# AlexanderKazakov/gcm

Hardware: AMD Instinct MI355X
Metric: Mnode-steps/sec + achieved HBM GB/s, 3D isotropic elastic 512³ CubicGrid (higher is better)
Workload: dtype f64; 1 GPU; 3-D isotropic elastic CubicGrid 512^3, borderSize 2, Courant 0.9, tau 0.9, one full time step (3 stages); global_nodes=134217728, slabs=1, launch=single process, parallelism=single, fp=fma

## Files before the change

gcm_amd/csrc/iso.hpp:

```cpp
#pragma once

#include "common.hpp"
#include "launch.hpp"

namespace gcmx {


__host__ __device__ constexpr int sig3(int i, int j) {
	return (i <= j) ? 3 + (i * 3 - ((i - 1) * i) / 2 + j - i)
	                : 3 + (j * 3 - ((j - 1) * j) / 2 + i - j);
}
__host__ __device__ constexpr unsigned bit(int i) { return 1u << i; }

__host__ __device__ constexpr int tang1(int s) { return s == 0 ? 1 : 0; }
__host__ __device__ constexpr int tang2(int s) { return s == 2 ? 1 : 2; }
__host__ __device__ constexpr int sgn1(int s) { return s == 0 ? -1 : 1; }
__host__ __device__ constexpr int sgn2(int s) { return s == 2 ? 1 : -1; }

enum Slot : int { kZero = 0, kOne, kHalf, kA, kB, kG, kP1, kP2, kS };
struct Coef {
	int slot;
	int sign;
};
__host__ __device__ constexpr Coef cz() { return Coef{kZero, 0}; }
// ... 3 lines not shown
	const int ss = sig3(S, S), st1 = sig3(t1, S), st2 = sig3(t2, S);
	const int s11 = sig3(t1, t1), s22 = sig3(t2, t2), s12 = sig3(t1, t2);
	return (k == 0) ? (j == S ? Coef{kOne, 1} : j == ss ? Coef{kA, 1} : cz())
	     : (k == 1) ? (j == S ? Coef{kOne, 1} : j == ss ? Coef{kA, -1} : cz())
	     : (k == 2) ? (j == t1 ? Coef{kOne, s1} : j == st1 ? Coef{kB, s1} : cz())
	     : (k == 3) ? (j == t1 ? Coef{kOne, s1} : j == st1 ? Coef{kB, -s1} : cz())
	     : (k == 4) ? (j == t2 ? Coef{kOne, s2} : j == st2 ? Coef{kB, s2} : cz())
	     : (k == 5) ? (j == t2 ? Coef{kOne, s2} : j == st2 ? Coef{kB, -s2} : cz())
	     : (k == 6) ? (j == s12 ? Coef{kOne, s1 * s2} : cz())
	     : (k == 7) ? (j == s11 ? Coef{kOne, 1} : j == s22 ? Coef{kOne, -1} : cz())
	                : (j == s11 ? Coef{kOne, 1} : j == s22 ? Coef{kOne, 1}
	                   : j == ss ? Coef{kG, 1} : cz());
}

__host__ __device__ constexpr Coef iso_u1(int S, int c, int n) {
	const int t1 = tang1(S), t2 = tang2(S), s1 = sgn1(S), s2 = sgn2(S);
	const int ss = sig3(S, S), st1 = sig3(t1, S), st2 = sig3(t2, S);
	const int s11 = sig3(t1, t1), s22 = sig3(t2, t2), s12 = sig3(t1, t2);
	return (n == 0) ? (c == S ? Coef{kHalf, 1} : c == ss ? Coef{kP1, 1}
	                   : (c == s11 || c == s22) ? Coef{kP2, 1} : cz())
	     : (n == 1) ? (c == S ? Coef{kHalf, 1} : c == ss ? Coef{kP1, -1}
	                   : (c == s11 || c == s22) ? Coef{kP2, -1} : cz())
	     : (n == 2) ? (c == t1 ? Coef{kHalf, s1} : c == st1 ? Coef{kS, s1} : cz())
	     : (n == 3) ? (c == t1 ? Coef{kHalf, s1} : c == st1 ? Coef{kS, -s1} : cz())
	     : (n == 4) ? (c == t2 ? Coef{kHalf, s2} : c == st2 ? Coef{kS, s2} : cz())
	     : (n == 5) ? (c == t2 ? Coef{kHalf, s2} : c == st2 ? Coef{kS, -s2} : cz())
	     : (n == 6) ? (c == s12 ? Coef{kOne, s1 * s2} : cz())
	     : (n == 7) ? (c == s11 ? Coef{kHalf, 1} : c == s22 ? Coef{kHalf, -1} : cz())
	                : (c == s11 ? Coef{kHalf, 1} : c == s22 ? Coef{kHalf, 1} : cz());
}

__host__ __device__ constexpr unsigned iso_window(int S) {
	unsigned m = 0;
	for (int k = 0; k < 6; k++)
		for (int j = 0; j < 9; j++)
			if (iso_u(S, k, j).slot != kZero) m |= bit(j);
	return m;
}
__host__ __device__ constexpr unsigned iso_center_only(int S) {
	unsigned m = 0;
	for (int k = 6; k < 9; k++)
		for (int j = 0; j < 9; j++)
			if (iso_u(S, k, j).slot != kZero) m |= bit(j);
	return m & ~iso_window(S);
}
__host__ __device__ constexpr int wslot(unsigned mask, int j) {
	int n = 0;
	for (int i = 0; i < j; i++) n += (mask >> i) & 1u;
	return n;
}
__host__ __device__ constexpr int popc9(unsigned m) {
	int n = 0;
	for (int i = 0; i < 9; i++) n += (m >> i) & 1u;
	return n;
}
template <int SLOT, int SIGN>
__device__ __forceinline__ double term(const IsoAxis& A, double v) {
	double m;
	if constexpr (SLOT == kOne) m = v;
	else if constexpr (SLOT == kHalf) m = v * 0.5;
	else if constexpr (SLOT == kA) m = A.a * v;
	else if constexpr (SLOT == kB) m = A.b * v;
	else if constexpr (SLOT == kG) m = A.g * v;
	else if constexpr (SLOT == kP1) m = A.p1 * v;
	else if constexpr (SLOT == kP2) m = A.p2 * v;
	else m = A.s * v;
	return SIGN > 0 ? m : -m;
}

template <int S, bool ISU1, int ROW, int J = 0>
struct RowSum {
	template <class F>
	__device__ __forceinline__ static double go(const IsoAxis& A, F val, double acc, bool first) {
		if constexpr (J == 9) {
			return acc;
		} else {
			constexpr Coef c = ISU1 ? iso_u1(S, ROW, J) : iso_u(S, ROW, J);
			if constexpr (c.slot == kZero) {
				return RowSum<S, ISU1, ROW, J + 1>::go(A, val, acc, first);
			} else {
				const double t = term<c.slot, c.sign>(A, val(J));
				return RowSum<S, ISU1, ROW, J + 1>::go(A, val, first ? t : acc + t, false);
			}
		}
	}
};

__host__ __device__ constexpr int pair_vel(int S, int P) { return P == 0 ? S : P == 1 ? tang1(S) : tang2(S); }
__host__ __device__ constexpr int pair_sig(int S, int P) {
	return P == 0 ? sig3(S, S) : P == 1 ? sig3(tang1(S), S) : sig3(tang2(S), S);
}

#ifndef GCMX_FMA
#define GCMX_FMA 0
#endif
#ifndef GCMX_LAGRANGE
#define GCMX_LAGRANGE GCMX_FMA
#endif
template <int BS>
__device__ __forceinline__ double lagrange_minmax(const double (&s)[BS + 1], const double* __restrict__ w) {
	double ans = s[0] * w[0];
#pragma unroll
	for (int i = 1; i <= BS; i++) ans = __builtin_fma(w[i], s[i], ans);
	return vlimit(ans, s[0], s[1]);
}

template <int S, int BS, bool KF0, int P, class WF>
__device__ __forceinline__ void pair_update(const IsoAxis& A, WF W, double& ra, double& rb) {
	const double* coef = (P == 0) ? A.c1 : A.c2;
	const double* wts = (P == 0) ? A.w1 : A.w2;
	const int kf = (P == 0) ? A.kf1 : A.kf2;
	auto interp = [&](int j, int sh) {
		double sv[BS + 1];
#pragma unroll
		for (int i = 0; i <= BS; i++) sv[i] = W(j, sh * i);
		if constexpr (GCMX_LAGRANGE && KF0 && BS <= 2) return lagrange_minmax<BS>(sv, wts);
		else return newton_minmax<BS, KF0>(sv, kf, coef);
	};
	ra = RowSum<S, false, 2 * P>::go(A, [&](int j) { return interp(j, -1); }, 0.0, true);
	rb = RowSum<S, false, 2 * P + 1>::go(A, [&](int j) { return interp(j, 1); }, 0.0, true);
}

template <int S, class CF>
__device__ __forceinline__ void center_update(const IsoAxis& A, CF C, double (&r)[9]) {
	r[6] = RowSum<S, false, 6>::go(A, C, 0.0, true);
	r[7] = RowSum<S, false, 7>::go(A, C, 0.0, true);
	r[8] = RowSum<S, false, 8>::go(A, C, 0.0, true);
}

template <int S>
__device__ __forceinline__ void u1_apply(const IsoAxis& A, const double (&r)[9], double (&out)[9]) {
	auto rv = [&](int n) { return r[n]; };
	out[0] = RowSum<S, true, 0>::go(A, rv, 0.0, true);
	out[1] = RowSum<S, true, 1>::go(A, rv, 0.0, true);
	out[2] = RowSum<S, true, 2>::go(A, rv, 0.0, true);
	out[3] = RowSum<S, true, 3>::go(A, rv, 0.0, true);
	out[4] = RowSum<S, true, 4>::go(A, rv, 0.0, true);
	out[5] = RowSum<S, true, 5>::go(A, rv, 0.0, true);
	out[6] = RowSum<S, true, 6>::go(A, rv, 0.0, true);
	out[7] = RowSum<S, true, 7>::go(A, rv, 0.0, true);
	out[8] = RowSum<S, true, 8>::go(A, rv, 0.0, true);
}

template <int S, int BS, bool KF0, class WF, class CF>
__device__ __forceinline__ void node_update(const IsoAxis& A, WF W, CF C, double (&out)[9]) {
	double r[9];
	pair_update<S, BS, KF0, 0>(A, W, r[0], r[1]);
	pair_update<S, BS, KF0, 1>(A, W, r[2], r[3]);
	pair_update<S, BS, KF0, 2>(A, W, r[4], r[5]);
	center_update<S>(A, C, r);
	u1_apply<S>(A, r, out);
}

typedef const __attribute__((address_space(1))) double* gcptr;
typedef __attribute__((address_space(1))) double* gptr;
#ifndef GCMX_SGPR_BASES
#define GCMX_SGPR_BASES 1
#endif
__device__ __forceinline__ gcptr sgpr_ptr(const double* p) {
	gcptr q = (gcptr)p;
#if GCMX_SGPR_BASES
	asm volatile("" : "+s"(q));
#endif
	return q;
}
__device__ __forceinline__ gptr sgpr_ptr(double* p) {
	gptr q = (gptr)p;
#if GCMX_SGPR_BASES
	asm volatile("" : "+s"(q));
#endif
	return q;
}
struct Planes {
	gcptr b[kMaxM];
	__device__ __forceinline__ Planes(const double* p, long long cs) {
#pragma unroll
		for (int j = 0; j < kMaxM; j++) b[j] = sgpr_ptr(p + j * cs);
	}
	__device__ __forceinline__ double ld(int j, unsigned off) const {
		typedef const __attribute__((address_space(1))) char* gcb;
		return *reinterpret_cast<gcptr>(reinterpret_cast<gcb>(b[j]) + (size_t)(off << 3));
	}
};
struct PlanesW {
	gptr b[kMaxM];
	__device__ __forceinline__ PlanesW(double* p, long long cs) {
#pragma unroll
		for (int j = 0; j < kMaxM; j++) b[j] = sgpr_ptr(p + j * cs);
	}
	__device__ __forceinline__ void st(int j, unsigned off, double v) const {
		typedef __attribute__((address_space(1))) char* gb;
		*reinterpret_cast<gptr>(reinterpret_cast<gb>(b[j]) + (size_t)(off << 3)) = v;
	}
	__device__ __forceinline__ void st_nt(int j, unsigned off, double v) const {
		typedef __attribute__((address_space(1))) char* gb;
		__builtin_nontemporal_store(v, reinterpret_cast<gptr>(reinterpret_cast<gb>(b[j]) + (size_t)(off << 3)));
	}
};

__device__ __forceinline__ unsigned opaque_u32(unsigned x) {
	asm("" : "+v"(x));
	return x;
}
__device__ __forceinline__ double ld_b(const Planes& p, int j, unsigned boff) {
	typedef const __attribute__((address_space(1))) char* gcb;
	return *reinterpret_cast<gcptr>(reinterpret_cast<gcb>(p.b[j]) + (unsigned long long)boff);
}
__device__ __forceinline__ double ld_nt_b(const Planes& p, int j, unsigned boff) {
	typedef const __attribute__((address_space(1))) char* gcb;
	return __builtin_nontemporal_load(reinterpret_cast<gcptr>(reinterpret_cast<gcb>(p.b[j]) + (unsigned long long)boff));
}
__device__ __forceinline__ void st_b(const PlanesW& p, int j, unsigned boff, double v) {
	typedef __attribute__((address_space(1))) char* gb;
	*reinterpret_cast<gptr>(reinterpret_cast<gb>(p.b[j]) + (unsigned long long)boff) = v;
}
__device__ __forceinline__ void st_nt_b(const PlanesW& p, int j, unsigned boff, double v) {
	typedef __attribute__((address_space(1))) char* gb;
	__builtin_nontemporal_store(v, reinterpret_cast<gptr>(reinterpret_cast<gb>(p.b[j]) + (unsigned long long)boff));
}

typedef double dpair __attribute__((ext_vector_type(2)));
__device__ __forceinline__ dpair ld2_b(const Planes& p, int j, unsigned boff) {
	typedef const __attribute__((address_space(1))) char* gcb;
	typedef const __attribute__((address_space(1))) dpair* gcp2;
	return *reinterpret_cast<gcp2>(reinterpret_cast<gcb>(p.b[j]) + (unsigned long long)boff);
}
__device__ __forceinline__ dpair ld2_nt_b(const Planes& p, int j, unsigned boff) {
	typedef const __attribute__((address_space(1))) char* gcb;
	typedef const __attribute__((address_space(1))) dpair* gcp2;
	return __builtin_nontemporal_load(reinterpret_cast<gcp2>(reinterpret_cast<gcb>(p.b[j]) + (unsigned long long)boff));
}
__device__ __forceinline__ void st2_b(const PlanesW& p, int j, unsigned boff, dpair v) {
	typedef __attribute__((address_space(1))) char* gb;
	typedef __attribute__((address_space(1))) dpair* gp2;
	*reinterpret_cast<gp2>(reinterpret_cast<gb>(p.b[j]) + (unsigned long long)boff) = v;
}
__device__ __forceinline__ void st2_nt_b(const PlanesW& p, int j, unsigned boff, dpair v) {
	typedef __attribute__((address_space(1))) char* gb;
	typedef __attribute__((address_space(1))) dpair* gp2;
	__builtin_nontemporal_store(v, reinterpret_cast<gp2>(reinterpret_cast<gb>(p.b[j]) + (unsigned long long)boff));
}
__device__ __forceinline__ void half_swap(double& a, double& b) {
	typedef unsigned u32x2 __attribute__((ext_vector_type(2)));
	const u32x2 x = __builtin_bit_cast(u32x2, a), y = __builtin_bit_cast(u32x2, b);
	const u32x2 lo = __builtin_amdgcn_permlane32_swap(x.x, y.x, false, false);
	const u32x2 hi = __builtin_amdgcn_permlane32_swap(x.y, y.y, false, false);
	a = __builtin_bit_cast(double, u32x2{lo.x, hi.x});
	b = __builtin_bit_cast(double, u32x2{lo.y, hi.y});
}

}
```

gcm_amd/csrc/kernels_xyz.hip:

```cpp
#include "iso.hpp"

#include <cstring>
#include <string>
#include <type_traits>

namespace gcmx {
#ifndef GCMX_FMA
#define GCMX_FMA 0
#endif
#if GCMX_FMA
#define GCMX_XYZ_NS xyz_fma
#define GCMX_FP_TAG ", FMA"
#else
#define GCMX_XYZ_NS xyz_exact
#define GCMX_FP_TAG ""
#endif
namespace GCMX_XYZ_NS {


#ifndef GCMX_XYZ_MINWAVES
#define GCMX_XYZ_MINWAVES 4
#endif
#ifndef GCMX_XYZ_CHUNK
#define GCMX_XYZ_CHUNK 128
// ... 111 lines not shown
	};
#pragma unroll
	for (int k = 0; k < W; k++) {
		const int r = yb - BS + k;
		double xr[9];
		if (r >= 0 && r < Y) {
			PairWin wa;
			x_load_a(wa, r);
			x_stage_rest(wa, r, xr);
		} else {
#pragma unroll
			for (int j = 0; j < 9; j++) xr[j] = 0.0;
		}
		push(xr, k);
	}
	auto clamp_row = [&](int r) { return r < Y + BS - 1 ? r : Y + BS - 1; };
	const unsigned zo = live ? (unsigned)z : (unsigned)Z;

	int buf = 0;
#pragma unroll GCMX_XYZ_UNROLL
	for (int y = yb; y < ye; y++) {
		double yv[9];
		node_update<1, BS, KF0>(
		    AY, [&](int j, int o) { return win[wslot(WMY, j)][BS + o]; },
		    [&](int j) { return ((WMY >> j) & 1u) ? win[wslot(WMY, j)][BS] : cen[0][wslot(CMY, j)]; },
		    yv);
#pragma unroll
		for (int j = 0; j < 9; j++)
			if ((WMZ >> j) & 1u) lds[buf][wslot(WMZ, j)][BS + z] = live ? yv[j] : 0.0;
		PairWin wa_next;
		__syncthreads();
		{
			double zv[9];
			node_update<2, BS, KF0>(
			    AZ, [&](int j, int o) { return lds[buf][wslot(WMZ, j)][BS + z + o]; },
			    [&](int j) { return ((WMZ >> j) & 1u) ? lds[buf][wslot(WMZ, j)][BS + z] : yv[j]; }, zv);
			const unsigned offo = plane + (unsigned)y * sty + zo;
			sched_fence();
			x_load_a(wa_next, clamp_row(y + BS + 1));
			sched_fence();
#pragma unroll
			for (int c = 0; c < 9; c++) out_p.st_nt(c, offo, live ? zv[c] : 0.0);
		}
		buf ^= 1;
#pragma unroll
		for (int q = 0; q < NWY; q++)
#pragma unroll
			for (int o = 0; o < W - 1; o++) win[q][o] = win[q][o + 1];
#pragma unroll
		for (int k = 0; k < BS; k++)
#pragma unroll
			for (int q = 0; q < (NCY > 0 ? NCY : 1); q++) cen[k][q] = cen[k + 1][q];
		{
			double xr[9];
			sched_fence();
			x_stage_rest(wa_next, clamp_row(y + BS + 1), xr);
			push(xr, W - 1);
			sched_fence();
		}
	}
}


#ifndef GCMX_TX2_MINWAVES
#define GCMX_TX2_MINWAVES 2
#endif
#ifndef GCMX_TX2_ZS2
#define GCMX_TX2_ZS2 -1
#endif
#ifndef GCMX_TX2_NB
#define GCMX_TX2_NB 1
#endif
#ifndef GCMX_TX2_SLEEP
#define GCMX_TX2_SLEEP 1
#endif
#ifndef GCMX_TX2_BUF
#define GCMX_TX2_BUF 1
#endif
#ifndef GCMX_TX2_PROBE_NOX
#define GCMX_TX2_PROBE_NOX 0
#endif
#ifndef GCMX_TX2_DIAG
#define GCMX_TX2_DIAG 0
#endif
#if GCMX_TX2_DIAG
__device__ unsigned long long g_tx2_diag[16][8];
#define TX2_T(i)                                                      \
	do {                                                              \
		const unsigned long long now_ = __builtin_amdgcn_s_memtime(); \
		dt_[i] += now_ - tprev_;                                      \
		tprev_ = now_;                                                \
	} while (0)
#else
#define TX2_T(i) \
	do {         \
	} while (0)
#endif
#ifndef GCMX_TX2_GEN2_DEFAULT
#define GCMX_TX2_GEN2_DEFAULT 64
#endif
#ifndef GCMX_TX2_PRIO
#define GCMX_TX2_PRIO 0
#endif
#if GCMX_TX2_PRIO
#define TX2_PRIO_HI() __builtin_amdgcn_s_setprio(GCMX_TX2_PRIO)
#define TX2_PRIO_LO() __builtin_amdgcn_s_setprio(0)
#else
#define TX2_PRIO_HI() \
	do {              \
	} while (0)
#define TX2_PRIO_LO() \
	do {              \
	} while (0)
#endif
#ifndef GCMX_TX2_ZPERM
#define GCMX_TX2_ZPERM 1
#endif
#ifndef GCMX_TX2_BLKT
#define GCMX_TX2_BLKT 0
#endif
#if GCMX_TX2_BLKT
constexpr int kBlkMax = 8192;
__device__ unsigned long long g_tx2_blk[kBlkMax][8][2];
__device__ unsigned g_tx2_hw[kBlkMax];
#endif

#ifndef GCMX_TX2_FACEMAP
#define GCMX_TX2_FACEMAP 1
#endif
#ifndef GCMX_TX2_FACE_LDS
#define GCMX_TX2_FACE_LDS 0
#endif
#ifndef GCMX_TX2_STNT
#define GCMX_TX2_STNT 1
#endif
#ifndef GCMX_TX2_ALT
#define GCMX_TX2_ALT 1
#endif
#ifndef GCMX_TX2_NTOUTER
#define GCMX_TX2_NTOUTER 0
#endif
#ifndef GCMX_TX2_NTLOAD
#define GCMX_TX2_NTLOAD 1
#endif
#ifndef GCMX_HET_AB
#define GCMX_HET_AB 0
#endif
#ifndef GCMX_ZS_PAIRS_FIRST
#define GCMX_ZS_PAIRS_FIRST 1
#endif

#ifndef GCMX_TX2_WIDE
#define GCMX_TX2_WIDE 1
#endif
#ifndef GCMX_TX2_UNROLL
#define GCMX_TX2_UNROLL 1
#endif



__host__ __device__ constexpr int wcomp(unsigned mask, int q) {
	int n = 0;
	for (int j = 0; j < 9; j++)
		if ((mask >> j) & 1u) {
			if (n == q) return j;
			n++;
		}
	return -1;
}

template <int BS, int ZT, bool KF0, bool UNI, bool FACES, bool HET, bool ZS = false, bool WD = false>
__global__ __launch_bounds__(ZT, GCMX_TX2_MINWAVES) void k_step_tx2(
    const double* __restrict__ in, double* __restrict__ outl, Geo g, IsoAxis AX, IsoAxis AY_,
    IsoAxis AZ_, int x0, int chunk, int nplanes, int xb0, int nplanesb, FaceBC fb,
    const IsoAxis* __restrict__ mtab, const uint8_t* __restrict__ mat) {
	static_assert(!HET || (KF0 && UNI), "heterogeneous step: floor(q) = 0, Z == ZT, equal axes");
	static_assert(!ZS || (UNI && !HET), "z split: uniform medium");
	const IsoAxis& AY = UNI ? AX : AY_;
	const IsoAxis& AZ = UNI ? AX : AZ_;
	constexpr unsigned WMX = iso_window(0);
	constexpr unsigned CMX = iso_center_only(0);
	constexpr int NCX = popc9(CMX);
	constexpr unsigned WMY = iso_window(1);
	constexpr unsigned CMY = iso_center_only(1);
	constexpr int NWY = popc9(WMY);
	constexpr int NCY = popc9(CMY);
	constexpr unsigned WMZ = iso_window(2);
	constexpr int NWZ = popc9(WMZ);
	constexpr int W = 2 * BS + 1;
	constexpr int WX = W + 1;
	constexpr int LW = ZT + 2 * BS;
	static_assert(NCX >= 1 && NCY >= 1, "isotropic structure");
	constexpr bool NB = UNI && GCMX_TX2_NB;
	constexpr int NW = ZT / 64;
	static_assert(!NB || ZT % 64 == 0, "NB needs whole waves");
	constexpr bool WIDE = WD && NB && GCMX_TX2_WIDE && GCMX_TX2_BUF;
	static_assert(!WD || WIDE, "wide instance launched without its path compiled in");
	constexpr int RW = WIDE ? 68 : 64 + 2 * BS;
	constexpr bool ZS2 = GCMX_TX2_ZS2 < 0 ? !NB : GCMX_TX2_ZS2 != 0;
	__shared__ double zl[NB ? 1 : 2][NB ? 1 : NWZ][NB ? 1 : LW];
	__shared__ double rg[NB ? NW : 1][NB ? 2 : 1][NB ? NWZ : 1][NB ? RW : 1];
	__shared__ double eg[NB ? 2 : 1][NB ? NW : 1][2][NB ? 2 : 1][NB ? NWZ : 1][BS];
	__shared__ int rdy[NB ? NW : 1];
	__shared__ double cl[BS + 1][2][NCY][ZT];
	__shared__ IsoAxis hlds[HET ? kHetMaxMaterials : 1];
	__shared__ double hode[HET ? kHetMaxMaterials : 1];
	__shared__ double flds[FACES && GCMX_TX2_FACE_LDS ? 4 : 1][9];

#if GCMX_TX2_ZPERM
	const int z = [] {
		int w = __builtin_amdgcn_readfirstlane((int)(threadIdx.x >> 6));
		if constexpr (ZT == 512) w = w < 4 ? 2 * w : 2 * (w - 4) + 1;
		const int l = (int)(threadIdx.x & 63);
		return w * 64 + (WIDE ? ((l & 31) << 1) | (l >> 5) : l);
	}();
#else
	const int z = WIDE ? (int)((threadIdx.x & ~63u) | ((threadIdx.x & 31u) << 1) | ((threadIdx.x >> 5) & 1u)) : (int)threadIdx.x;
#endif
#if GCMX_TX2_BLKT
	const unsigned long long blk_t0_ = __builtin_amdgcn_s_memrealtime();
#endif
	const int Y = g.sizes[1], Z = g.sizes[2];
	int x, yb, ye, xbeg, xend;
	bool rev;
	int zp = 0;
	const int nz = ZS ? g.sizes[2] / ZT : 1;
	{
		const int pa = (g.gx0 + x0) & 1, pb = (g.gx0 + xb0) & 1;
		const int npa = (nplanes + pa + 1) / 2;
		const int npair = npa + (nplanesb > 0 ? (nplanesb + pb + 1) / 2 : 0);
		const int T = (int)gridDim.x, b = (int)blockIdx.x;
		int p = xcd_order(b, T);
		if constexpr (ZS && !GCMX_ZS_PAIRS_FIRST) {
			zp = p % nz;
			p /= nz;
		}
		int q = p % npair;
		int cidx = p / npair;
		if (!ZS && chunk < 0) {
			const int co = (-chunk) & 0xFFFF, half = T >> 4;
			const int j = b >> 3, gen = j >= half ? 1 : 0;
			const int G = (b & 7) * half + (j - gen * half);
			const int ncg = (T >> 1) / npair;
			q = G % npair;
			cidx = G / npair + gen * ncg;
			const int cy = (-chunk) >> 16;
			auto start = [&](int c) { return c <= ncg ? c * co : ncg * co + (c - ncg) * cy; };
			yb = start(cidx);
			ye = min(start(cidx + 1), Y);
		}
		x = q < npa ? x0 - pa + 2 * q : xb0 - pb + 2 * (q - npa);
		xbeg = q < npa ? x0 : xb0;
		xend = q < npa ? x0 + nplanes : xb0 + nplanesb;
		if constexpr (ZS && GCMX_ZS_PAIRS_FIRST) {
			zp = cidx % nz;
			cidx /= nz;
		}
		if (ZS || chunk > 0) {
			yb = cidx * chunk;
			ye = min(yb + chunk, Y);
		}
		rev = GCMX_TX2_ALT && (cidx & 1);
	}
	const bool one = x >= xbeg;
	const bool two = x + 1 < xend;
	const bool live = UNI || z < Z;
	const int zc = live ? z : Z - 1;
	const unsigned stx = (unsigned)g.stride[0];
	const unsigned sty = (unsigned)g.stride[1];
	const long long pbase = (long long)x * g.stride[0];
	const unsigned plane = (unsigned)g.origin;
	const unsigned zo = live ? (unsigned)z : (unsigned)Z;
#if GCMX_TX2_BUF
	const Planes src(in + pbase, g.cs);
	const PlanesW out_p(outl + pbase, g.cs);
	const unsigned zpart = ZS ? (unsigned)(zp * ZT) : 0u;
	const int zg = (int)zpart + zc;
	const unsigned lv = (zpart + (unsigned)zc) * 8u, sv = (zpart + zo) * 8u;
	const unsigned pxm = plane - (unsigned)BS * stx;
	auto ldx = [&](int j, int k, int r) {
#if GCMX_TX2_PROBE_NOX
		k = k < BS ? BS : (k > BS + 1 ? BS + 1 : k);
#endif
		const int d = (k == WX - 1 && !two) ? 2 * BS : (k == 0 && !one) ? 1 : k;
		if (GCMX_TX2_NTOUTER && (k == 0 || k == WX - 1))
			return ld_nt_b(src, j, opaque_u32(lv + (pxm + (unsigned)d * stx + (unsigned)r * sty) * 8u));
		return ld_b(src, j, opaque_u32(lv + (pxm + (unsigned)d * stx + (unsigned)r * sty) * 8u));
	};
	auto ldc = [&](int j, int k, int r) {
		if constexpr (!GCMX_TX2_NTLOAD) return ldx(j, k, r);
		const int d = (k == WX - 1 && !two) ? 2 * BS : (k == 0 && !one) ? 1 : k;
		return ld_nt_b(src, j, opaque_u32(lv + (pxm + (unsigned)d * stx + (unsigned)r * sty) * 8u));
	};
	auto stz = [&](int c, int t, int y, double v) {
		const unsigned o = opaque_u32(sv + (plane + (unsigned)t * stx + (unsigned)y * sty) * 8u);
		if constexpr (GCMX_TX2_STNT) st_nt_b(out_p, c, o, v);
		else st_b(out_p, c, o, v);
	};
	const bool hsel = (threadIdx.x & 32u) != 0;
	const unsigned lw = (zpart + (unsigned)(z & ~63) + 2u * (threadIdx.x & 31u)) * 8u;
	auto ldw = [&](int j, int ka, int kb, int r, bool nt) {
		auto cl_ = [&](int k) { return (k == WX - 1 && !two) ? 2 * BS : (k == 0 && !one) ? 1 : k; };
		const unsigned pa = (pxm + (unsigned)cl_(ka) * stx) * 8u, pb = (pxm + (unsigned)cl_(kb) * stx) * 8u;
		const unsigned o = opaque_u32(lw + (hsel ? pb : pa) + (unsigned)r * sty * 8u);
		return nt ? ld2_nt_b(src, j, o) : ld2_b(src, j, o);
	};
	auto stw = [&](int c, int y, double v0, double v1) {
		const unsigned o = opaque_u32(lw + (plane + (hsel ? stx : 0u) + (unsigned)y * sty) * 8u);
		const dpair v = {v0, v1};
		if constexpr (GCMX_TX2_STNT) st2_nt_b(out_p, c, o, v);
		else st2_b(out_p, c, o, v);
	};
#else
	const unsigned base = plane + zc;
	const Planes src(in + pbase, g.cs);
	const PlanesW out_p(outl + pbase, g.cs);
	auto ldx = [&](int j, int k, int r) {
		const int d = (k == WX - 1 && !two) ? BS : (k == 0 && !one) ? 1 - BS : k - BS;
		return src.ld(j, base + (unsigned)r * sty + (unsigned)d * stx);
	};
	auto ldc = [&](int j, int k, int r) { return ldx(j, k, r); };
	auto stz = [&](int c, int t, int y, double v) { out_p.st_nt(c, plane + (unsigned)y * sty + zo + (unsigned)t * stx, v); };
#endif
	auto mt = [&](unsigned k) -> const IsoAxis& {
		if constexpr (GCMX_HET_AB >= 1) return AX;
		return hlds[k];
	};
	auto two_v = [&](int f, int j) -> double {
		if constexpr (FACES && GCMX_TX2_FACE_LDS) return flds[f][j];
		return fb.two_v[f][j];
	};
	struct GhostRule {
		unsigned mask;
		bool none;
		double two[9];
	};
	auto ghost_rule = [&](int f, int t, int pos, unsigned need) -> GhostRule {
		GhostRule r;
		r.none = false;
		if (GCMX_TX2_FACEMAP && fb.map[f]) {
			const int xx = (t == 1 && !two) ? x : (t == 0 && !one) ? x + 1 : x + t;
			const unsigned c = fb.map[f][(size_t)xx * (f < 2 ? Z : Y) + pos];
			r.none = c == kNoFaceCond;
			const FaceCond& fc = fb.conds[r.none ? 0u : c];
			r.mask = r.none ? 0u : fc.mask;
#pragma unroll
			for (int j = 0; j < 9; j++)
				if ((need >> j) & 1u) r.two[j] = r.none ? 0.0 : fc.two_v[j];
		} else {
			r.mask = fb.mask[f];
#pragma unroll
			for (int j = 0; j < 9; j++)
				if ((need >> j) & 1u) r.two[j] = two_v(f, j);
		}
		return r;
	};
	auto ghost = [](const GhostRule& r, int j, double v) -> double {
		return r.none ? 0.0 : ((r.mask >> j) & 1u) ? -v + r.two[j] : v;
	};

	const int wv = z >> 6, ln = z & 63;
	const bool seam_own = ZS && ((zp > 0 && z < BS) || (zp < nz - 1 && z >= ZT - BS));
	auto rs = [](int c) { return WIDE ? (c >> 1) + ((c & 1) ? 35 : 1) : BS + c; };
	const int rs0 = rs(ln), rs1 = rs(ln + 1);
	auto rso = [&](int o) { return !WIDE ? rs0 + o : (o & 1) ? rs1 + ((o - 1) >> 1) : rs0 + (o >> 1); };
	const bool seam_pair = [&] {
		const int cb = (z & ~63) + 2 * (int)(threadIdx.x & 31u);
		auto sc = [&](int c) { return (zp > 0 && c < BS) || (zp < nz - 1 && c >= ZT - BS); };
		return ZS && sc(cb) && sc(cb + 1);
	}();
	const int ci = WIDE ? (int)threadIdx.x : z;
	if constexpr (NB) {
		if (ln < BS || ln >= 64 - BS) {
			const int hs = rs(ln < BS ? ln - BS : ln + BS);
#pragma unroll
			for (int t = 0; t < 2; t++)
#pragma unroll
				for (int q = 0; q < NWZ; q++) rg[wv][t][q][hs] = 0.0;
		}
		if (z < NW) rdy[z] = -1;
		__syncthreads();
	} else if (z < 2 * BS) {
		const int gslot = (z < BS) ? z : (Z + z);
#pragma unroll
		for (int t = 0; t < 2; t++)
#pragma unroll
			for (int q = 0; q < NWZ; q++) zl[t][q][gslot] = 0.0;
	}

	typedef double PairWin[2][WX];
	auto pair_load = [&](auto PC, PairWin& w, int r) {
		constexpr int P = decltype(PC)::value;
		if constexpr (WIDE) {
#if GCMX_TX2_BUF
#pragma unroll
			for (int m = 0; m < WX / 2; m++) {
				const dpair a = ldw(pair_vel(0, P), 2 * m, 2 * m + 1, r, false);
				const dpair b = ldw(pair_sig(0, P), 2 * m, 2 * m + 1, r, false);
				w[0][2 * m] = a.x, w[0][2 * m + 1] = a.y;
				w[1][2 * m] = b.x, w[1][2 * m + 1] = b.y;
			}
#endif
			return;
		}
#pragma unroll
		for (int k = 0; k < WX; k++) {
			w[0][k] = ldx(pair_vel(0, P), k, r);
			w[1][k] = ldx(pair_sig(0, P), k, r);
		}
	};
	auto pair_fix = [&](const PairWin& w, PairWin& u) {
#pragma unroll
		for (int v = 0; v < 2; v++) {
#pragma unroll
			for (int k = 0; k < WX; k++) u[v][k] = w[v][k];
			if constexpr (WIDE) {
#pragma unroll
				for (int m = 0; m < WX / 2; m++) half_swap(u[v][2 * m], u[v][2 * m + 1]);
			}
		}
	};
	auto pair_rows = [&](auto PC, const PairWin& w, double (&rr)[2][9], const IsoAxis& A0, const IsoAxis& A1,
	                     bool same) {
		constexpr int P = decltype(PC)::value;
		if (KF0 && !same) {
#pragma unroll
			for (int t = 0; t < 2; t++)
				pair_update<0, BS, true, P>(
				    t ? A1 : A0, [&](int j, int o) { return j == pair_vel(0, P) ? w[0][t + BS + o] : w[1][t + BS + o]; },
				    rr[t][2 * P], rr[t][2 * P + 1]);
		} else if constexpr (KF0 && !GCMX_LAGRANGE) {
			const IsoAxis& AS = A0;
			const double* c = (P == 0) ? AS.c1 : AS.c2;
			double im[2][2], ip[2][2];
#pragma unroll
			for (int v = 0; v < 2; v++) {
				double D[BS + 1][WX];
#pragma unroll
				for (int k = 0; k < WX; k++) D[0][k] = w[v][k];
#pragma unroll
				for (int i = 1; i <= BS; i++)
#pragma unroll
					for (int k = 0; k + i < WX; k++) D[i][k] = (D[i - 1][k + 1] - D[i - 1][k]) * c[i - 1];
#pragma unroll
				for (int t = 0; t < 2; t++) {
					const int m = t + BS;
					double a = D[0][m], b = D[0][m];
#pragma unroll
					for (int i = 1; i <= BS; i++) {
						a += D[i][m];
						b = (i % 2) ? b - D[i][m - i] : b + D[i][m - i];
					}
					ip[v][t] = vlimit(a, D[0][m], D[0][m + 1]);
					im[v][t] = vlimit(b, D[0][m], D[0][m - 1]);
				}
			}
#pragma unroll
			for (int t = 0; t < 2; t++) {
				rr[t][2 * P] = RowSum<0, false, 2 * P>::go(
				    AS, [&](int j) { return j == pair_vel(0, P) ? im[0][t] : im[1][t]; }, 0.0, true);
				rr[t][2 * P + 1] = RowSum<0, false, 2 * P + 1>::go(
				    AS, [&](int j) { return j == pair_vel(0, P) ? ip[0][t] : ip[1][t]; }, 0.0, true);
			}
		} else {
#pragma unroll
			for (int t = 0; t < 2; t++)
				pair_update<0, BS, KF0, P>(
				    t ? A1 : A0, [&](int j, int o) { return j == pair_vel(0, P) ? w[0][t + BS + o] : w[1][t + BS + o]; },
				    rr[t][2 * P], rr[t][2 * P + 1]);
		}
	};
	auto sched_fence = [] { __builtin_amdgcn_sched_barrier(0); };
	using P0 = std::integral_constant<int, 0>;
	using P1 = std::integral_constant<int, 1>;
	using P2 = std::integral_constant<int, 2>;
	struct XPre {
		PairWin a, b;
	};
	auto cv_load = [&](double (&cv)[2][9], int r) {
		if constexpr (WIDE) {
#if GCMX_TX2_BUF
#pragma unroll
			for (int j = 0; j < 9; j++)
				if ((CMX >> j) & 1u) {
					const dpair v = ldw(j, BS, BS + 1, r, GCMX_TX2_NTLOAD != 0);
					cv[0][j] = v.x, cv[1][j] = v.y;
				}
#endif
			return;
		}
#pragma unroll
		for (int t = 0; t < 2; t++)
#pragma unroll
			for (int j = 0; j < 9; j++)
				if ((CMX >> j) & 1u) cv[t][j] = ldc(j, BS + t, r);
	};
	auto x_load_ahead = [&](XPre& pre, int r) {
		pair_load(P0{}, pre.a, r);
		pair_load(P1{}, pre.b, r);
	};
	auto mat_of = [&](int t, int r) -> unsigned {
		const int xx = (t == 1 && !two) ? x : (t == 0 && !one) ? x + 1 : x + t;
		const int rr_ = r < 0 ? 0 : (r < Y ? r : Y - 1);
		return mat[((size_t)xx * Y + rr_) * Z + z];
	};
	auto x_compute = [&](const XPre& pre, const PairWin& wc_, const double (&cv_)[2][9], double (&xr)[2][9],
	                     const IsoAxis& A0, const IsoAxis& A1, bool same) {
		double rr[2][9], n0[2][9], cv[2][9];
		PairWin pa, pb, wc;
		pair_fix(pre.a, pa);
		pair_rows(P0{}, pa, rr, A0, A1, same);
		pair_fix(pre.b, pb);
		pair_rows(P1{}, pb, rr, A0, A1, same);
		sched_fence();
		pair_fix(wc_, wc);
		pair_rows(P2{}, wc, rr, A0, A1, same);
#pragma unroll
		for (int t = 0; t < 2; t++) {
			n0[t][pair_vel(0, 0)] = pa[0][t + BS];
			n0[t][pair_sig(0, 0)] = pa[1][t + BS];
			n0[t][pair_vel(0, 1)] = pb[0][t + BS];
			n0[t][pair_sig(0, 1)] = pb[1][t + BS];
			n0[t][pair_vel(0, 2)] = wc[0][t + BS];
			n0[t][pair_sig(0, 2)] = wc[1][t + BS];
		}
		sched_fence();
#pragma unroll
		for (int j = 0; j < 9; j++)
			if ((CMX >> j) & 1u) {
				cv[0][j] = cv_[0][j], cv[1][j] = cv_[1][j];
				if constexpr (WIDE) half_swap(cv[0][j], cv[1][j]);
			}
#pragma unroll
		for (int t = 0; t < 2; t++) {
			const IsoAxis& A = t ? A1 : A0;
			center_update<0>(A, [&](int j) { return ((WMX >> j) & 1u) ? n0[t][j] : cv[t][j]; }, rr[t]);
			u1_apply<0>(A, rr[t], xr[t]);
		}
	};
	auto key_of = [&](int r) -> unsigned {
		if constexpr (GCMX_HET_AB >= 2) return 0u;
		return mat_of(0, r) | (mat_of(1, r) << 8);
	};
	auto x_stage = [&](const XPre& pre, int r, double (&xr)[2][9], unsigned key) {
		PairWin wc;
		double cv[2][9];
		TX2_PRIO_HI();
		pair_load(P2{}, wc, r);
		cv_load(cv, r);
		TX2_PRIO_LO();
		sched_fence();
		if constexpr (HET) {
			const unsigned m0 = key & 255u, m1 = key >> 8;
			x_compute(pre, wc, cv, xr, mt(m0), mt(m1), m0 == m1);
		} else {
			x_compute(pre, wc, cv, xr, AX, AX, true);
		}
	};

	double win[2][NWY][W];
	unsigned hk[W];
#pragma unroll
	for (int k = 0; k < W; k++) hk[k] = 0;
	if constexpr (HET) {
		for (int i = z; i < kHetMaxMaterials * (int)(sizeof(IsoAxis) / 4); i += ZT)
			reinterpret_cast<unsigned*>(hlds)[i] = reinterpret_cast<const unsigned*>(mtab)[i];
		if (fb.ode_on && fb.ode_f && z < kHetMaxMaterials) hode[z] = fb.ode_f[z];
	}
	if constexpr (FACES && GCMX_TX2_FACE_LDS) {
#pragma unroll
		for (int c = 0; c < 36; c++)
			if (z == c) flds[c / 9][c % 9] = fb.two_v[c / 9][c % 9];
	}
	if constexpr (HET || (FACES && GCMX_TX2_FACE_LDS)) __syncthreads();
	auto run = [&](auto RV) {
	constexpr bool REV = decltype(RV)::value;
	constexpr int S = REV ? -1 : 1;
	auto cl_at = [&](int r) { return &cl[(r + 2 * BS + 2) % (BS + 1)][0][0][ci]; };
	auto push = [&](const double (&xr)[2][9], int slot, int r) {
		double* cp = cl_at(r);
#pragma unroll
		for (int t = 0; t < 2; t++)
#pragma unroll
			for (int j = 0; j < 9; j++) {
				if ((WMY >> j) & 1u) win[t][wslot(WMY, j)][slot] = xr[t][j];
				if ((CMY >> j) & 1u) cp[(t * NCY + wslot(CMY, j)) * ZT] = xr[t][j];
			}
	};
	auto mirror_slot = [&](int k, int ks, int f) {
#pragma unroll
		for (int t = 0; t < 2; t++) {
			const GhostRule gr = ghost_rule(f, t, zg, WMY);
#pragma unroll
			for (int q = 0; q < NWY; q++) {
				double v = 0.0;
#pragma unroll
				for (int kk = 0; kk < W; kk++)
					if (kk == ks) v = win[t][q][kk];
				const double gv = ghost(gr, wcomp(WMY, q), v);
#pragma unroll
				for (int kk = 0; kk < W; kk++)
					if (kk == k) win[t][q][kk] = gv;
			}
		}
	};
	const int y0 = REV ? ye - 1 : yb;
#pragma unroll
	for (int k = 0; k < W; k++) {
		const int r = y0 + S * (k - BS);
		double xr[2][9];
		if (r >= 0 && r < Y) {
			XPre pre;
			if constexpr (HET) hk[k] = key_of(r);
			x_load_ahead(pre, r);
			x_stage(pre, r, xr, hk[k]);
		} else {
#pragma unroll
			for (int t = 0; t < 2; t++)
#pragma unroll
				for (int j = 0; j < 9; j++) xr[t][j] = 0.0;
		}
		push(xr, k, r);
	}
	if constexpr (FACES) {
		if (fb.on & 3u) {
#pragma unroll
			for (int k = 0; k < W; k++) {
				const int r = y0 + S * (k - BS);
				const int f = r < 0 ? 0 : 1, ks = BS + S * ((r < 0 ? -r : 2 * (Y - 1) - r) - y0);
				if ((r < 0 || r >= Y) && ((fb.on >> f) & 1u) && ks >= 0 && ks < W) mirror_slot(k, ks, f);
			}
		}
	}
	auto clamp_row = [&](int r) {
		if constexpr (REV) return r > -BS ? r : -BS;
		return r < Y + BS - 1 ? r : Y + BS - 1;
	};

#if GCMX_TX2_DIAG
	unsigned long long dt_[8] = {0, 0, 0, 0, 0, 0, 0, 0};
	unsigned long long tprev_ = __builtin_amdgcn_s_memtime();
#endif
	auto y_stage = [&](int y, double (&yv)[2][9]) {
		const double* cp = cl_at(y);
#pragma unroll
		for (int t = 0; t < 2; t++) {
			auto go = [&](const IsoAxis& A) {
				node_update<1, BS, KF0>(
				    A, [&](int j, int o) { return win[t][wslot(WMY, j)][BS + S * o]; },
				    [&](int j) { return ((WMY >> j) & 1u) ? win[t][wslot(WMY, j)][BS] : cp[(t * NCY + wslot(CMY, j)) * ZT]; },
				    yv[t]);
			};
			if constexpr (HET) go(mt(t ? hk[BS] >> 8 : hk[BS] & 255u));
			else go(AY);
		}
	};
	auto z_ghosts = [&](int y, const double (&yv)[2][9], auto&& put) {
		const int wu = __builtin_amdgcn_readfirstlane(z >> 6);
#pragma unroll
		for (int side = 0; side < 2; side++) {
			const int Zl = ZS ? ZT : Z;
			if (ZS && (side ? zp != nz - 1 : zp != 0)) continue;
			const int lo = side ? Zl - 1 - BS : 1, hi = side ? Zl - 2 : BS;
			if (!((fb.on >> (2 + side)) & 1u) || wu * 64 > hi || wu * 64 + 63 < lo) continue;
			if (z < lo || z > hi) continue;
#pragma unroll
			for (int t = 0; t < 2; t++) {
				const GhostRule gr = ghost_rule(2 + side, t, y, WMZ);
#pragma unroll
				for (int j = 0; j < 9; j++)
					if ((WMZ >> j) & 1u) put(side, t, wslot(WMZ, j), ghost(gr, j, yv[t][j]));
			}
		}
	};
	auto publish = [&](int it, int y, const double (&yv)[2][9]) {
		const int es = it & 1;
		if constexpr (NB) {
			double* egp = ln < BS ? &eg[es][wv][0][0][0][ln] : &eg[es][wv][1][0][0][ln - (64 - BS)];
			const bool edge = ln < BS || ln >= 64 - BS;
			asm volatile("" ::: "memory");
#pragma unroll
			for (int t = 0; t < 2; t++)
#pragma unroll
				for (int j = 0; j < 9; j++)
					if ((WMZ >> j) & 1u) {
						const int q = wslot(WMZ, j);
						rg[wv][t][q][rs0] = yv[t][j];
						if (edge) egp[(t * NWZ + q) * BS] = yv[t][j];
					}
			if constexpr (FACES)
				z_ghosts(y, yv, [&](int side, int t, int q, double v) {
					if (side == 0) rg[0][t][q][rs(-z)] = v;
					else rg[NW - 1][t][q][rs(2 * ((ZS ? ZT : Z) - 1) - z - 64 * (NW - 1))] = v;
				});
			asm volatile("s_waitcnt lgkmcnt(0)" ::: "memory");
			__hip_atomic_store(&rdy[wv], it, __ATOMIC_RELAXED, __HIP_MEMORY_SCOPE_WORKGROUP);
		} else {
			__syncthreads();
#pragma unroll
			for (int t = 0; t < 2; t++)
#pragma unroll
				for (int j = 0; j < 9; j++)
					if ((WMZ >> j) & 1u) {
						const int q = wslot(WMZ, j);
						if constexpr (FACES) {
							if (UNI || z < Z || z >= Z + BS) zl[t][q][BS + z] = live ? yv[t][j] : 0.0;
						} else {
							zl[t][q][BS + z] = live ? yv[t][j] : 0.0;
						}
					}
			if constexpr (FACES)
				z_ghosts(y, yv, [&](int side, int t, int q, double v) {
					if (side == 0) zl[t][q][BS - z] = v;
					else zl[t][q][BS + 2 * (Z - 1) - z] = v;
				});
			__syncthreads();
		}
	};
	auto collect = [&](int it) {
		if constexpr (NB && NW > 1) {
			const int es = it & 1;
			for (;;) {
				const int a = wv > 0 ? __hip_atomic_load(&rdy[wv - 1], __ATOMIC_RELAXED, __HIP_MEMORY_SCOPE_WORKGROUP) : it;
				const int b =
				    wv < NW - 1 ? __hip_atomic_load(&rdy[wv + 1], __ATOMIC_RELAXED, __HIP_MEMORY_SCOPE_WORKGROUP) : it;
				if (__builtin_amdgcn_readfirstlane(min(a, b)) >= it) break;
				if constexpr (GCMX_TX2_SLEEP > 0) __builtin_amdgcn_s_sleep(GCMX_TX2_SLEEP);
			}
			asm volatile("" ::: "memory");
			if (ln < BS && wv > 0) {
#pragma unroll
				for (int t = 0; t < 2; t++)
#pragma unroll
					for (int q = 0; q < NWZ; q++) rg[wv][t][q][rs(ln - BS)] = eg[es][wv - 1][1][t][q][ln];
			}
			if (ln >= 64 - BS && wv < NW - 1) {
#pragma unroll
				for (int t = 0; t < 2; t++)
#pragma unroll
					for (int q = 0; q < NWZ; q++) rg[wv][t][q][rs(ln + BS)] = eg[es][wv + 1][0][t][q][ln - (64 - BS)];
			}
			asm volatile("" ::: "memory");
		}
	};
	auto z_stage_store = [&](int t, int y, const double (&yv)[2][9], double (&zv)[9]) {
		auto go = [&](const IsoAxis& A) {
			if constexpr (NB)
				node_update<2, BS, KF0>(
				    A, [&](int j, int o) { return rg[wv][t][wslot(WMZ, j)][rso(o)]; },
				    [&](int j) { return ((WMZ >> j) & 1u) ? rg[wv][t][wslot(WMZ, j)][rs0] : yv[t][j]; }, zv);
			else
				node_update<2, BS, KF0>(
				    A, [&](int j, int o) { return zl[t][wslot(WMZ, j)][BS + z + o]; },
				    [&](int j) { return ((WMZ >> j) & 1u) ? zl[t][wslot(WMZ, j)][BS + z] : yv[t][j]; }, zv);
		};
		if constexpr (HET) go(mt(t ? hk[BS] >> 8 : hk[BS] & 255u));
		else go(AZ);
		if (fb.ode_on) {
			double f = fb.ode;
			if constexpr (HET)
				if (fb.ode_f) f = hode[t ? hk[BS] >> 8 : hk[BS] & 255u];
#pragma unroll
			for (int c = 3; c < 9; c++) zv[c] = zv[c] * f;
		}
		if constexpr (WIDE) return;
		if ((t == 0 ? one : two) && !(ZS && seam_own)) {
#pragma unroll
			for (int c = 0; c < 9; c++) stz(c, t, y, live ? zv[c] : 0.0);
		}
	};
	auto z_store_wide = [&](int y, double (&zv)[2][9]) {
#if GCMX_TX2_BUF
#pragma unroll
		for (int c = 0; c < 9; c++) half_swap(zv[0][c], zv[1][c]);
		if ((hsel ? two : one) && !seam_pair) {
#pragma unroll
			for (int c = 0; c < 9; c++) stw(c, y, zv[0][c], zv[1][c]);
		}
#endif
	};
	auto x_enter = [&](int y, const XPre& pre, unsigned kn) {
#pragma unroll
		for (int t = 0; t < 2; t++)
#pragma unroll
			for (int q = 0; q < NWY; q++)
#pragma unroll
				for (int o = 0; o < W - 1; o++) win[t][q][o] = win[t][q][o + 1];
		if constexpr (HET) {
#pragma unroll
			for (int o = 0; o < W - 1; o++) hk[o] = hk[o + 1];
			hk[W - 1] = kn;
		}
		double xr[2][9];
		sched_fence();
		const int r = y + S * (BS + 1);
		x_stage(pre, clamp_row(r), xr, kn);
		push(xr, W - 1, r);
		sched_fence();
		if constexpr (FACES) {
			const int f = r < 0 ? 0 : 1;
			if ((r < 0 || r >= Y) && ((fb.on >> f) & 1u)) {
				const int ks = BS + S * ((r < 0 ? -r : 2 * (Y - 1) - r) - (y + S));
				if (ks >= 0 && ks < W) mirror_slot(W - 1, ks, f);
			}
		}
	};
	auto row = [&](int y, int it) {
		double yv[2][9], zv[2][9];
		XPre pre;
		const int rn = clamp_row(y + S * (BS + 1));
		unsigned kn = 0;
		if constexpr (HET) kn = key_of(rn);
		y_stage(y, yv);
		TX2_T(0);
		publish(it, y, yv);
		TX2_T(2);
		if constexpr (ZS2) {
			sched_fence();
			pair_load(P0{}, pre.a, rn);
			sched_fence();
		} else {
			sched_fence();
			TX2_PRIO_HI();
			x_load_ahead(pre, rn);
			TX2_PRIO_LO();
			sched_fence();
		}
		TX2_T(6);
		collect(it);
		TX2_T(4);
#pragma unroll
		for (int t = 0; t < 2; t++) {
			if constexpr (ZS2) {
				if (t == 1) {
					sched_fence();
					pair_load(P1{}, pre.b, rn);
					sched_fence();
				}
			}
			z_stage_store(t, y, yv, zv[t]);
		}
		if constexpr (WIDE) z_store_wide(y, zv);
		TX2_T(3);
		x_enter(y, pre, kn);
		TX2_T(5);
	};
#if GCMX_TX2_UNROLL > 1
#pragma unroll GCMX_TX2_UNROLL
#endif
	for (int it = 0; it < ye - yb; it++) row(REV ? ye - 1 - it : yb + it, it);
#if GCMX_TX2_BLKT
	if ((threadIdx.x & 63) == 0 && blockIdx.x < (unsigned)kBlkMax && threadIdx.x < 512) {
		const unsigned long long t1 = __builtin_amdgcn_s_memrealtime();
		g_tx2_blk[blockIdx.x][threadIdx.x / 64][0] = blk_t0_;
		g_tx2_blk[blockIdx.x][threadIdx.x / 64][1] = t1;
		if (threadIdx.x == 0) g_tx2_hw[blockIdx.x] = __builtin_amdgcn_s_getreg((31 << 11) | 4);
	}
#endif
#if GCMX_TX2_DIAG
	if ((threadIdx.x & 63) == 0) {
		const int wv = threadIdx.x / 64;
		for (int i = 0; i < 8; i++) atomicAdd(&g_tx2_diag[wv][i], dt_[i]);
	}
#endif
	};
	if (rev) run(std::true_type{});
	else run(std::false_type{});
}

template <int BS, bool KF0, bool FACES>
__global__ __launch_bounds__(256) void k_zseam(const double* __restrict__ in, double* __restrict__ outl, Geo g,
                                                IsoAxis A, int x0, int nplanes, int xb0, int nplanesb, int zt,
                                                int chunk, FaceBC fb) {
	const unsigned ode_on = fb.ode_on;
	const double ode = fb.ode;
	constexpr int NC = 4 * BS, PB = 256 / NC, W = 2 * BS + 1;
	const int Y = g.sizes[1], ncut = g.sizes[2] / zt - 1;
	const int nch = (Y + chunk - 1) / chunk;
	int b = (int)blockIdx.x;
	const int ch = b % nch;
	b /= nch;
	const int cut = b % ncut;
	const int pg = b / ncut;
	const int c = (int)threadIdx.x % NC, xi = pg * PB + (int)threadIdx.x / NC;
	const bool valid = xi < nplanes + nplanesb;
	const int x = !valid ? x0 : xi < nplanes ? x0 + xi : xb0 + (xi - nplanes);
	const int z = (cut + 1) * zt - 2 * BS + c;
	const long long stx = g.stride[0], sty = g.stride[1], cs = g.cs;
	const long long base = g.origin + (long long)x * stx + z;
	const int yb = ch * chunk, ye = min(yb + chunk, Y);
	auto xstage = [&](int r, double (&xr)[9]) {
		const int rc = r < -BS ? -BS : (r > Y + BS - 1 ? Y + BS - 1 : r);
		const long long o = base + (long long)rc * sty;
		node_update<0, BS, KF0>(
		    A, [&](int j, int oo) { return in[j * cs + o + oo * stx]; }, [&](int j) { return in[j * cs + o]; }, xr);
	};
	double win[9][W];
	auto mirror = [&](int k, int ks, int f) {
		unsigned mask;
		bool none = false;
		double two[9];
		if (fb.map[f]) {
			const unsigned cnd = fb.map[f][(size_t)x * g.sizes[2] + z];
			none = cnd == kNoFaceCond;
			const FaceCond& fc = fb.conds[none ? 0u : cnd];
			mask = none ? 0u : fc.mask;
#pragma unroll
			for (int j = 0; j < 9; j++) two[j] = none ? 0.0 : fc.two_v[j];
		} else {
			mask = fb.mask[f];
#pragma unroll
			for (int j = 0; j < 9; j++) two[j] = fb.two_v[f][j];
		}
#pragma unroll
		for (int j = 0; j < 9; j++) {
			double v = 0.0;
#pragma unroll
			for (int kk = 0; kk < W; kk++)
				if (kk == ks) v = win[j][kk];
			const double gv = none ? 0.0 : ((mask >> j) & 1u) ? -v + two[j] : v;
#pragma unroll
			for (int kk = 0; kk < W; kk++)
				if (kk == k) win[j][kk] = gv;
		}
	};
#pragma unroll
	for (int k = 0; k < W; k++) {
		double xr[9];
		const int r = yb - BS + k;
		if (r >= 0 && r < Y) xstage(r, xr);
		else
#pragma unroll
			for (int j = 0; j < 9; j++) xr[j] = 0.0;
#pragma unroll
		for (int j = 0; j < 9; j++) win[j][k] = xr[j];
	}
	if constexpr (FACES) {
		if (fb.on & 3u) {
#pragma unroll
			for (int k = 0; k < W; k++) {
				const int r = yb - BS + k;
				const int f = r < 0 ? 0 : 1, ks = BS + ((r < 0 ? -r : 2 * (Y - 1) - r) - yb);
				if ((r < 0 || r >= Y) && ((fb.on >> f) & 1u) && ks >= 0 && ks < W) mirror(k, ks, f);
			}
		}
	}
	const bool mine = valid && c >= BS && c < 3 * BS;
	const int lane = (int)(threadIdx.x & 63);
	for (int y = yb; y < ye; y++) {
		double yv[9], zv[9];
		node_update<1, BS, KF0>(A, [&](int j, int o) { return win[j][BS + o]; }, [&](int j) { return win[j][BS]; }, yv);
		node_update<2, BS, KF0>(
		    A, [&](int j, int o) { return __shfl(yv[j], lane + o, 64); }, [&](int j) { return yv[j]; }, zv);
		if (mine) {
			if (ode_on) {
#pragma unroll
				for (int k = 3; k < 9; k++) zv[k] = zv[k] * ode;
			}
			const long long off = base + (long long)y * sty;
#pragma unroll
			for (int k = 0; k < 9; k++) __builtin_nontemporal_store(zv[k], outl + k * cs + off);
		}
#pragma unroll
		for (int j = 0; j < 9; j++)
#pragma unroll
			for (int k = 0; k < W - 1; k++) win[j][k] = win[j][k + 1];
		double xr[9];
		const int r = y + BS + 1;
		if (r < Y) xstage(r, xr);
		else
#pragma unroll
			for (int j = 0; j < 9; j++) xr[j] = 0.0;
#pragma unroll
		for (int j = 0; j < 9; j++) win[j][W - 1] = xr[j];
		if constexpr (FACES) {
			if (r >= Y && ((fb.on >> 1) & 1u)) {
				const int ks = BS + (2 * (Y - 1) - r) - (y + 1);
				if (ks >= 0 && ks < W) mirror(W - 1, ks, 1);
			}
		}
	}
}


static bool same_axis(const IsoAxis& p, const IsoAxis& q) {
	static_assert(sizeof(IsoAxis) == 18 * 8 + 2 * 4, "IsoAxis has padding");
	return std::memcmp(&p, &q, sizeof(IsoAxis)) == 0;
}

template <int BS, int ZT, bool KF0, bool UNI, bool FACES, bool HET, bool ZS = false, bool WD = false>
static const char* tx2_name() {
	static const std::string s = "k_step_tx2<" + std::to_string(BS) + ", " + std::to_string(ZT) + ", " +
	                             (KF0 ? "KF0" : "!KF0") + ", " + (UNI ? "UNI" : "!UNI") + ", " +
	                             (FACES ? "FACES" : "!FACES") + (HET ? ", HET" : "") + (ZS ? ", ZS" : "") +
	                             (UNI && !WD ? ", N8" : "") + GCMX_FP_TAG + ">";
// ... 266 lines not shown
```

Before: 37630 Mnode-steps/s.

## Split wide z-stage update into independent output groups stored incrementally

Decomposes the z-axis node update into four groups (pairs 0..2 plus centre rows) whose outputs form disjoint component sets, and computes and stores each group separately in the wide path. Live ranges shrink because only a subset of the nine outputs per half is held at once, which is meant to cut register pressure and let stores overlap with later groups' math. It can optionally read the centre window values from the y-stage registers instead of LDS. The cost is some repeated LDS reads and ODE scaling per group, and the ZS2 pair_load interleave is dropped in this path.

```diff
diff --git a/gcm_amd/csrc/iso.hpp b/gcm_amd/csrc/iso.hpp
--- a/gcm_amd/csrc/iso.hpp
+++ b/gcm_amd/csrc/iso.hpp
@@ -179,6 +179,49 @@
 	u1_apply<S>(A, r, out);
 }
 
+constexpr int kIsoGroups = 4;
+__host__ __device__ constexpr unsigned iso_group_rows(int G) {
+	return G == 0 ? bit(0) | bit(1) | bit(7) | bit(8) : G == 1 ? bit(2) | bit(3) : G == 2 ? bit(4) | bit(5) : bit(6);
+}
+__host__ __device__ constexpr unsigned iso_group_out(int S, int G) {
+	unsigned m = 0;
+	for (int c = 0; c < 9; c++)
+		for (int n = 0; n < 9; n++)
+			if (iso_u1(S, c, n).slot != kZero && ((iso_group_rows(G) >> n) & 1u)) m |= bit(c);
+	return m;
+}
+__host__ __device__ constexpr bool iso_groups_partition(int S) {
+	unsigned all = 0;
+	for (int G = 0; G < kIsoGroups; G++) {
+		if (all & iso_group_out(S, G)) return false;
+		all |= iso_group_out(S, G);
+	}
+	return all == 0x1FFu;
+}
+static_assert(iso_groups_partition(0) && iso_groups_partition(1) && iso_groups_partition(2), "isotropic structure");
+
+template <int S, int BS, bool KF0, int G, class WF, class CF>
+__device__ __forceinline__ void node_update_group(const IsoAxis& A, WF W, CF C, double (&out)[9]) {
+	double r[9] = {0.0, 0.0, 0.0, 0.0, 0.0, 0.0, 0.0, 0.0, 0.0};
+	if constexpr (G < 3) pair_update<S, BS, KF0, G>(A, W, r[2 * G], r[2 * G + 1]);
+	if constexpr (G == 0) {
+		r[7] = RowSum<S, false, 7>::go(A, C, 0.0, true);
+		r[8] = RowSum<S, false, 8>::go(A, C, 0.0, true);
+	}
+	if constexpr (G == 3) r[6] = RowSum<S, false, 6>::go(A, C, 0.0, true);
+	constexpr unsigned OM = iso_group_out(S, G);
+	auto rv = [&](int n) { return r[n]; };
+	if constexpr (OM & bit(0)) out[0] = RowSum<S, true, 0>::go(A, rv, 0.0, true);
+	if constexpr (OM & bit(1)) out[1] = RowSum<S, true, 1>::go(A, rv, 0.0, true);
+	if constexpr (OM & bit(2)) out[2] = RowSum<S, true, 2>::go(A, rv, 0.0, true);
+	if constexpr (OM & bit(3)) out[3] = RowSum<S, true, 3>::go(A, rv, 0.0, true);
+	if constexpr (OM & bit(4)) out[4] = RowSum<S, true, 4>::go(A, rv, 0.0, true);
+	if constexpr (OM & bit(5)) out[5] = RowSum<S, true, 5>::go(A, rv, 0.0, true);
+	if constexpr (OM & bit(6)) out[6] = RowSum<S, true, 6>::go(A, rv, 0.0, true);
+	if constexpr (OM & bit(7)) out[7] = RowSum<S, true, 7>::go(A, rv, 0.0, true);
+	if constexpr (OM & bit(8)) out[8] = RowSum<S, true, 8>::go(A, rv, 0.0, true);
+}
+
 typedef const __attribute__((address_space(1))) double* gcptr;
 typedef __attribute__((address_space(1))) double* gptr;
 #ifndef GCMX_SGPR_BASES
diff --git a/gcm_amd/csrc/kernels_xyz.hip b/gcm_amd/csrc/kernels_xyz.hip
--- a/gcm_amd/csrc/kernels_xyz.hip
+++ b/gcm_amd/csrc/kernels_xyz.hip
@@ -287,6 +287,9 @@
 
 #ifndef GCMX_TX2_WIDE
 #define GCMX_TX2_WIDE 1
+#endif
+#ifndef GCMX_TX2_ZGROUP
+#define GCMX_TX2_ZGROUP 1
 #endif
 #ifndef GCMX_TX2_UNROLL
 #define GCMX_TX2_UNROLL 1
@@ -332,7 +335,10 @@
 	constexpr bool WIDE = WD && NB && GCMX_TX2_WIDE && GCMX_TX2_BUF;
 	static_assert(!WD || WIDE, "wide instance launched without its path compiled in");
 	constexpr int RW = WIDE ? 68 : 64 + 2 * BS;
-	constexpr bool ZS2 = GCMX_TX2_ZS2 < 0 ? !NB : GCMX_TX2_ZS2 != 0;
+	constexpr bool ZGROUP = WIDE && GCMX_TX2_ZGROUP != 0;
+	constexpr bool ZG_BIG_FIRST = GCMX_TX2_ZGROUP == 2 || GCMX_TX2_ZGROUP == 4;
+	constexpr bool ZG_YV = GCMX_TX2_ZGROUP <= 2 && BS == 2;
+	constexpr bool ZS2 =GCMX_TX2_ZS2 < 0 ? !NB : GCMX_TX2_ZS2 != 0;
 	__shared__ double zl[NB ? 1 : 2][NB ? 1 : NWZ][NB ? 1 : LW];
 	__shared__ double rg[NB ? NW : 1][NB ? 2 : 1][NB ? NWZ : 1][NB ? RW : 1];
 	__shared__ double eg[NB ? 2 : 1][NB ? NW : 1][2][NB ? 2 : 1][NB ? NWZ : 1][BS];
@@ -609,6 +615,7 @@
 	using P0 = std::integral_constant<int, 0>;
 	using P1 = std::integral_constant<int, 1>;
 	using P2 = std::integral_constant<int, 2>;
+	using P3 = std::integral_constant<int, 3>;
 	struct XPre {
 		PairWin a, b;
 	};
@@ -911,6 +918,44 @@
 		if ((hsel ? two : one) && !seam_pair) {
 #pragma unroll
 			for (int c = 0; c < 9; c++) stw(c, y, zv[0][c], zv[1][c]);
+		}
+#endif
+	};
+	auto z_group_store = [&](auto GC, int y, const double (&yv)[2][9]) {
+#if GCMX_TX2_BUF
+		constexpr int G = decltype(GC)::value;
+		constexpr unsigned OM = iso_group_out(2, G);
+		double zv[2][9];
+#pragma unroll
+		for (int t = 0; t < 2; t++) {
+			auto go = [&](const IsoAxis& A) {
+				node_update_group<2, BS, KF0, G>(
+				    A, [&](int j, int o) { return (ZG_YV && o == 0) ? yv[t][j] : rg[wv][t][wslot(WMZ, j)][rso(o)]; },
+				    [&](int j) { return (!ZG_YV && ((WMZ >> j) & 1u)) ? rg[wv][t][wslot(WMZ, j)][rs0] : yv[t][j]; },
+				    zv[t]);
+			};
+			if constexpr (HET) go(mt(t ? hk[BS] >> 8 : hk[BS] & 255u));
+			else go(AZ);
+		}
+		if (fb.ode_on) {
+			sched_fence();
+#pragma unroll
+			for (int t = 0; t < 2; t++) {
+				double f = fb.ode;
+				if constexpr (HET)
+					if (fb.ode_f) f = hode[t ? hk[BS] >> 8 : hk[BS] & 255u];
+#pragma unroll
+				for (int c = 3; c < 9; c++)
+					if ((OM >> c) & 1u) zv[t][c] = zv[t][c] * f;
+			}
+		}
+#pragma unroll
+		for (int c = 0; c < 9; c++)
+			if ((OM >> c) & 1u) half_swap(zv[0][c], zv[1][c]);
+		if ((hsel ? two : one) && !seam_pair) {
+#pragma unroll
+			for (int c = 0; c < 9; c++)
+				if ((OM >> c) & 1u) stw(c, y, zv[0][c], zv[1][c]);
 		}
 #endif
 	};
@@ -964,18 +1009,26 @@
 		TX2_T(6);
 		collect(it);
 		TX2_T(4);
-#pragma unroll
-		for (int t = 0; t < 2; t++) {
-			if constexpr (ZS2) {
-				if (t == 1) {
-					sched_fence();
-					pair_load(P1{}, pre.b, rn);
-					sched_fence();
+		if constexpr (ZGROUP) {
+			if constexpr (ZG_BIG_FIRST) z_group_store(P0{}, y, yv);
+			z_group_store(P3{}, y, yv);
+			z_group_store(P1{}, y, yv);
+			z_group_store(P2{}, y, yv);
+			if constexpr (!ZG_BIG_FIRST) z_group_store(P0{}, y, yv);
+		} else {
+#pragma unroll
+			for (int t = 0; t < 2; t++) {
+				if constexpr (ZS2) {
+					if (t == 1) {
+						sched_fence();
+						pair_load(P1{}, pre.b, rn);
+						sched_fence();
+					}
 				}
-			}
-			z_stage_store(t, y, yv, zv[t]);
-		}
-		if constexpr (WIDE) z_store_wide(y, zv);
+				z_stage_store(t, y, yv, zv[t]);
+			}
+			if constexpr (WIDE) z_store_wide(y, zv);
+		}
 		TX2_T(3);
 		x_enter(y, pre, kn);
 		TX2_T(5);
```

New measurement: 38210 Mnode-steps/s, median of 5. No clear change (+1.5%).
